# countertype/brotli-lib

Measured on AMD Instinct MI355X. Metric: encode+decode MB/s at q11 lgwin=22, higher is better.
Workload: dtype u8; 1 GPU; C4 per-GPU shard: 1024 x 1048576 B enwik-style text, q11 lgwin22 GENERIC, encode -> decode round trip (statuses and sizes checked); streams_per_gpu=1024, quality=11, lgwin=22, mode=0, parallelism=shard1

## Files before the change

brotli-lib_amd/csrc/enc_common.h:

```cpp
#pragma once
#include <hip/hip_runtime.h>
#include <stdint.h>

#include "common.h"
#include "parts.h"

#ifndef RFC_CONST
#define RFC_CONST static __device__ const
#endif
#include "rfc_tables.h"

namespace mib {
namespace enc {

constexpr uint32_t kSegBits = 16;
constexpr uint32_t kSeg = 1u << kSegBits;
#ifndef MIB_MAX_MATCHES
#define MIB_MAX_MATCHES 4
#endif
constexpr int kMaxMatches = MIB_MAX_MATCHES;
static_assert(kMaxMatches == 4 || kMaxMatches == 6 || kMaxMatches == 8, "records of 4, 6 or 8 entries");
constexpr int kMatchRec = kMaxMatches;
constexpr uint32_t kMatchLenSat = 255;
constexpr int kLongCopy = 200;
// ... 387 lines not shown
                         const uint8_t *dict_data, uint32_t *matches);
void launch_cdict_matches(hipStream_t st, const Job *jobs, const uint32_t *pos_job, uint32_t total, uint32_t *matches);
void launch_find_matches(hipStream_t st, const Job *jobs, const uint32_t *pos_job, const SegRef *seg_ref,
                         const uint32_t *skeys, const uint32_t *svals, uint32_t total, int depth, uint32_t max_dist,
                         bool hist, bool parts, uint32_t *matches);
void launch_near_matches(hipStream_t st, const Job *jobs, const uint32_t *pos_job, const SegRef *seg_ref, uint32_t total,
                         uint32_t max_dist, bool hist, bool parts, uint32_t *matches);
void launch_lit_histo(hipStream_t st, const Job *jobs, const Seg *segs, int nsegs, uint32_t *lit_h);
void launch_hist_update(hipStream_t st, const Job *jobs, const uint32_t *pos_job, const uint32_t *skeys,
                        const uint32_t *svals, uint32_t total);
size_t cost_model_hist_bytes(int njobs);
void launch_cost_model(hipStream_t st, const Job *jobs, int njobs, const Seg *segs, int nsegs, const RawCmd *raw,
                       uint32_t *hist, CostModel *model);
void launch_dp(hipStream_t st, const Job *jobs, const Seg *segs, int nsegs, const uint32_t *lit_h, const CostModel *model,
               const uint32_t *matches, uint64_t *choice, bool cdict, bool font, const uint32_t *words, uint32_t *ring_hist,
               const Mb *mbs);
size_t dp_ring_hist_bytes(int nsegs);
void launch_any_binary(hipStream_t st, const Job *jobs, int njobs, uint32_t *flag);
void launch_words(hipStream_t st, const Job *jobs, const uint32_t *pos_job, const SegRef *seg_ref, uint32_t total, uint32_t *words);
void launch_backtrack(hipStream_t st, const Job *jobs, Seg *segs, int nsegs, const uint64_t *choice, RawCmd *raw);
void launch_carry(hipStream_t st, Job *jobs, int njobs, Seg *segs, const Mb *mbs);
void launch_derive_segs(hipStream_t st, const Seg *segs, int nsegs, uint32_t sample, Seg *d_sample, Seg *pieces);
void launch_merge_pieces(hipStream_t st, const Job *jobs, Seg *segs, int nsegs, const Seg *pieces, RawCmd *raw);
void launch_rep(hipStream_t st, const Job *jobs, Seg *segs, int nsegs, const CostModel *model, RawCmd *raw, uint32_t *cnts);
size_t sort_ws_bytes(uint32_t total);
void launch_sort(hipStream_t st, const Job *jobs, const uint32_t *pos_job, int njobs, uint32_t total, int hb, void *ws,
                 uint32_t *tmp_k, uint32_t *tmp_v, uint32_t *skeys, uint32_t *svals);
void launch_codes(hipStream_t st, const Job *jobs, const Seg *segs, const Mb *mbs, int nsegs, const RawCmd *raw, Cmd *cmds,
                  uint32_t *cmd_pos, Unit *units, uint32_t *unit_h);
void launch_split(hipStream_t st, hipStream_t side, const Job *jobs, Mb *mbs, int nmbs, Unit *units,
                  const uint32_t *unit_h, Codes *codes, int max_units, int max_short_units);
// ... 25 lines not shown
```

brotli-lib_amd/csrc/enc_parse.hip:

```cpp
#include <hipcub/hipcub.hpp>
#include <cstdlib>

#include "enc_common.h"

namespace mib {
namespace enc {

#ifdef MIB_PROF
__device__ unsigned long long g_dp_prof[8];
#define DPMARK(slot)                                  \
  do {                                                \
    const uint64_t t_ = __builtin_amdgcn_s_memtime(); \
    prof[slot] += t_ - pt0;                           \
    pt0 = t_;                                         \
  } while (0)
#define DPCOUNT(slot, v) prof[slot] += (v)
#else
#define DPMARK(slot) do {} while (0)
#define DPCOUNT(slot, v) do {} while (0)
#endif
constexpr int kDpWaves = 4;
constexpr int kLenTab = kLongCopy + 1;
constexpr int kInsTab = 256;
constexpr float kInf = 3.0e38f;
constexpr uint32_t kCostLast = 255;
#ifndef MIB_DP_OCC
#define MIB_DP_OCC 4
#endif
constexpr int kDpWavesPerSimd = MIB_DP_OCC;
#ifndef MIB_DP_OCC_KS4
#define MIB_DP_OCC_KS4 MIB_DP_OCC
#endif
constexpr int kPtabW = 20;
constexpr int kRepLen = 16;
static_assert(kLongCopy <= 325, "copy codes of lengths <= 325 are < 20 (command.ts getCopyLengthCode)");

typedef const __attribute__((address_space(1))) uint8_t GCU8;

__device__ __forceinline__ uint32_t copy_extra(int cc) { return cc < 8 ? 0u : cc < 18 ? (uint32_t)(cc - 6) >> 1 : cc < 23 ? (uint32_t)(cc - 12) : 24u; }
__device__ __forceinline__ uint32_t ins_extra(int ic) {
  return ic < 6 ? 0u : ic < 16 ? (uint32_t)(ic - 4) >> 1 : ic < 21 ? (uint32_t)(ic - 10) : ic == 21 ? 12u : ic == 22 ? 14u : 24u;
}
__device__ __forceinline__ float cmd_cost(int cmd) { return __builtin_amdgcn_logf(11.f + (float)cmd); }
__device__ __forceinline__ float dist_sym_cost(uint32_t code) { return __builtin_amdgcn_logf(20.f + (float)min(code, 127u)); }
__device__ __forceinline__ float cmd_price(int cmd, const CostModel *cm) { return cm ? cm->cmd[cmd] : cmd_cost(cmd); }
__device__ __forceinline__ float dist_price(uint32_t code, const CostModel *cm) {
  return cm ? cm->dist[min(code, 127u)] : dist_sym_cost(code);
// ... 41 lines not shown
__device__ __forceinline__ uint64_t choice_of(uint32_t d, uint32_t m) {
  const uint32_t cl = (m >> 16) ? 0u : m & 0xFFFF;
  return cl ? (((uint64_t)d << 32) | cl) : 0ull;
}
__device__ __forceinline__ uint32_t bperm(uint32_t lane_src, uint32_t v) {
  return (uint32_t)__builtin_amdgcn_ds_bpermute((int)(lane_src << 2), (int)v);
}
__device__ __forceinline__ uint32_t quad_entry0(uint32_t v) { return (uint32_t)__builtin_amdgcn_mov_dpp((int)v, 0x00, 0xF, 0xF, false); }
__device__ __forceinline__ uint32_t quad_entry1(uint32_t v) { return (uint32_t)__builtin_amdgcn_mov_dpp((int)v, 0x55, 0xF, 0xF, false); }
__device__ __forceinline__ uint32_t quad_shift1(uint32_t v) { return (uint32_t)__builtin_amdgcn_mov_dpp((int)v, 0x90, 0xF, 0xF, false); }

constexpr uint32_t kHistPos = 256;
static_assert(kHistPos > (uint32_t)kLongCopy, "a copy's predecessor must still be in the ring history");

template <int KS, bool KM, bool KD, bool KR, bool KC>
__global__ __launch_bounds__(64 * kDpWaves, KS == 4 ? MIB_DP_OCC_KS4 : (KC && KS == 2) ? 3 : kDpWavesPerSimd) void dp_kernel(const Job *jobs, const Seg *segs, int nsegs,
                                                           const uint32_t *lit_histo, const CostModel *model,
                                                           const uint32_t *matches,
                                                           uint64_t *choice , float cmd_pen, int use_rep,
                                                           const uint32_t *pwords, uint32_t *ring_hist, const Mb *mbs,
                                                           int kc_split) {
  constexpr int kS = KS;
  constexpr int kL = 64 / kS;
  constexpr int kC = (kL - 1 + kLongCopy) / kL + 1;
  static_assert(kL - 1 + kLongCopy < kL * kC, "every relaxed length must land in a chunk");
  static_assert(kRepLen <= kL, "a last-distance copy is measured by one lane per byte");
  static_assert(!KC || kL >= 16, "a lane per distance-cache candidate");
  constexpr uint64_t kLaneMask = kL == 64 ? ~0ull : ((1ull << kL) - 1);
  __shared__ uint32_t ptab_all[kDpWaves * kS][24 * kPtabW];
  __shared__ uint8_t cct_all[kL + kLenTab];
  uint8_t *const cctab = cct_all + kL;
  __shared__ uint16_t itab[kInsTab];
  __shared__ uint16_t litc_all[kDpWaves * kS][256];
  constexpr int kPadSh = KS == 4 ? 4 : 5;
  __shared__ StageEnt stg_all[kDpWaves][64 + (64 >> kPadSh)];
  for (int t = (int)threadIdx.x - kL; t < kLenTab; t += 64 * kDpWaves) cctab[t] = (uint8_t)(t >= 2 ? copy_code((uint32_t)t) : 0);
  for (int t = threadIdx.x; t < kInsTab; t += 64 * kDpWaves) {
    const int ic = ins_code((uint32_t)t);
    itab[t] = (uint16_t)(ic | (ins_extra(ic) << 8));
  }
  __syncthreads();
  const uint32_t lane = threadIdx.x & 63, w = (uint32_t)__builtin_amdgcn_readfirstlane((int)(threadIdx.x >> 6));
  const uint32_t h = lane / kL, hl = lane % kL, hbase = h * kL;
  const int sgi = (blockIdx.x * kDpWaves + (int)w) * kS + (int)h;
  StageEnt *stg = stg_all[w];
  uint16_t *litc = litc_all[w * kS + h];
  uint32_t *ptab = ptab_all[w * kS + h];
  uint32_t a = 0, b = 0, gbase = 0, job = 0;
  const uint8_t *data = nullptr;
  int ndirect = 0, npostfix = 0;
  uint32_t parts = 0, abs0 = 0, wabs = 0, pbits = 16, plag = 0, maxback = 0, cdl = 0;
  bool words = false;
  if (sgi < nsegs) {
    const Seg &sg = segs[sgi];
    const Job &jb = jobs[sg.job];
    a = sg.start;
    b = sg.end;
    gbase = jb.pos_base;
    job = sg.job;
    data = jb.data;
    ndirect = (int)jb.ndirect;
    npostfix = (int)jb.npostfix;
    parts = jb.parts;
    abs0 = jb.abs_base;
    wabs = jb.win_abs;
    pbits = jb.part_bits;
    plag = jb.part_lag;
    maxback = (1u << jb.lgwin) - 16;
    words = jb.dict != 0;
    cdl = jb.cdict ? jb.cdict_len : 0u;
  }
  if (kc_split && a < b && (mbs[segs[sgi].mb].ctx_mode == 2u) == KC) a = b;
  if (__ballot(a < b) == 0) return;
  const CostModel *cm = (KM && a < b) ? model + job : nullptr;
  const float dist0 = dist_price(0, cm);
  if (a < b)
    for (uint32_t t = hl; t < 24 * kPtabW; t += kL) {
      const int ic = (int)(t / kPtabW), cc = (int)(t % kPtabW);
      const _Float16 x = (_Float16)(copy_price(ic, cc, false, dist0, cm) + cmd_pen),
                     y = (_Float16)(copy_price(ic, cc, true, dist0, cm) + cmd_pen);
      ptab[t] = (uint32_t)__builtin_bit_cast(uint16_t, x) | ((uint32_t)__builtin_bit_cast(uint16_t, y) << 16);
    }
  if (cm) {
    if (a < b)
      for (uint32_t k = hl; k < 256; k += kL)
        litc[k] = (uint16_t)(uint32_t)(fminf(fmaxf(cm->lit[k], 1.f), 255.f) * 256.f);
  } else {
    uint32_t part = 0;
    if (a < b)
      for (uint32_t k = hl; k < 256; k += kL) part += lit_histo[job * 256 + k];
    for (int o = kL / 2; o; o >>= 1) part += __shfl_xor(part, o);
    const float lt = log2f((float)max(part, 1u));
    if (a < b)
      for (uint32_t k = hl; k < 256; k += kL) {
        const uint32_t c = lit_histo[job * 256 + k];
        const float v = c ? lt - log2f((float)c) : lt + 2.f;
        litc[k] = (uint16_t)(uint32_t)(fminf(fmaxf(v, 1.f), 255.f) * 256.f);
      }
  }
  wave_sync();
  float wc[kC];
  uint32_t wd[kC], wm[kC];
#pragma unroll
  for (int c = 0; c < kC; c++) {
    wc[c] = kInf;
    wd[c] = wm[c] = 0;
  }
  if (hl == 0) wc[0] = 0.f;
  Staged pf;
  uint32_t pf_at = a;
  if (a + hl < b) load_staged<KC>(pf, matches, data, pwords, gbase + a + hl, a + hl);
  uint32_t chd = 0, chm = 0;
  uint32_t rp_d = 0, rp_ic = 0, rp_cb = 0, rp_sb = 1;
  float rp_base = 0.f;
  const uint32_t cj = hl & 15u, rq = hl & 3u;
  const bool clane = KC && hl < 16u && (!KR || cj != 0u);
  const float ccost = KC ? dist_price(cj, cm) : 0.f;
  const uint32_t hoff = (uint32_t)sgi * (kHistPos * 4);
  uint32_t kf = 0;
  uint32_t kp_ld = 0, kp_h = 0;
  float kp_base = 0.f;
  uint32_t rg = 0;
// ... 3 lines not shown
  float cq_base = 0.f;
  auto words_on_ring = [&](uint32_t dd) { return words && is_dict(dd); };
  auto ring_step = [&](uint32_t kind, uint32_t dd, uint32_t h, uint32_t prev) -> uint32_t {
    const uint32_t v = kind == 2u ? h : prev;
    const uint32_t v0 = quad_entry0(v), vm = quad_shift1(v);
    const bool word = words_on_ring(dd);
    const bool push = kind == 2u && dd != v0 && !word;
    return push ? (rq == 0u ? dd : vm) : (kind == 2u && word && rq == 0u) ? dd : v;
  };
  uint32_t i = a, i0 = a;
  bool done = a >= b;
#ifdef MIB_PROF
  uint64_t prof[8] = {0, 0, 0, 0, 0, 0, 0, 0};
  uint64_t pt0 = __builtin_amdgcn_s_memtime();
#endif
  constexpr bool kEarly = KS == 4;
  auto stage = [&]() {
    Staged cur;
#pragma unroll
    for (int q = 0; q < kMaxMatches; q++) cur.m[q] = 0;
    cur.lit = 0;
    cur.w0 = cur.w1 = 0;
    if (pf_at == i0) {
      cur = pf;
    } else if (i0 + hl < b) {
      load_staged<KC>(cur, matches, data, pwords, gbase + i0 + hl, i0 + hl);
    }
    const uint32_t nx = i0 + kL;
    if constexpr (!kEarly) {
      if (nx + hl < b) load_staged<KC>(pf, matches, data, pwords, gbase + nx + hl, nx + hl);
    }
// ... 49 lines not shown
#pragma unroll
    for (int q = 0; kEarly && q < kMaxMatches; q++)
      if ((uint32_t)q < nm) {
        const float dc = (float)(dpq[q] >> 10) + dsc[q];
        e.mc[q] |= min((uint32_t)(dc * 4.f + 0.5f), kCostLast - 1) << 24;
      }
    e.info = (maxlen ? nm : 0u) | (maxlen << 8) | ((word ? maxlen : 2u) << 16);
    e.w[0] = KC ? cur.w0 : 0u;
    e.w[1] = KC ? cur.w1 : 0u;
    stg[lane + (lane >> kPadSh)] = e;
    if constexpr (kEarly) {
      if (nx + hl < b) load_staged<KC>(pf, matches, data, pwords, gbase + nx + hl, nx + hl);
    }
    pf_at = nx;
  };
  constexpr int kPre = kEarly ? 3 : 0;
  struct StepIn {
    uint32_t info;
    float lc;
    uint32_t m[kMaxMatches], mc[kMaxMatches];
    uint32_t cc[kPre ? kPre : 1];
  };
  auto read_step = [&](uint32_t o) {
    const uint32_t s = hbase + (o & (kL - 1));
    const StageEnt &e = stg[s + (s >> kPadSh)];
    StepIn r;
    r.info = e.info;
    r.lc = e.lc;
    if constexpr (kMaxMatches == 4) {
      const uint4 em = *reinterpret_cast<const uint4 *>(e.m), emc = *reinterpret_cast<const uint4 *>(e.mc);
      r.m[0] = em.x; r.m[1] = em.y; r.m[2] = em.z; r.m[3] = em.w;
// ... 93 lines not shown
          const uint32_t p = i0 + hl;
          if (p <= i && p != a) choice[gbase + p] = choice_of(chd, chm);
        }
        if (KC) {
          const uint32_t r1 = (kf & 3u) ? ring_step(kf & 3u, kp_ld, kp_h, rg) : rg;
          const bool ccopy = !(kf & 4u) && mm >= 2u && (mm >> 16) == 0u;
          const uint32_t hv = ccopy ? ring_hist[hoff + ((i - mm) & (kHistPos - 1)) * 4 + rq] : 0u;
          const uint32_t ri = ring_step(ccopy ? 2u : 1u, ld, hv, r1);
          rg = ring_step(2u, fd, ri, ri);
          kf = 4u;
        }
        i += fl;
        i0 = i;
        rp_d = 0;
#pragma unroll
        for (int c = 0; c < kC; c++) wc[c] = kInf;
        if (hl == 0) {
          wc[0] = fc;
          wd[0] = fd;
          wm[0] = fl;
        }
        stage();
      }
      wave_sync();
      DPMARK(2);
      continue;
    }
    const uint32_t actm = 0u - (uint32_t)act;
    uint32_t mL[kMaxMatches], vpk[kMaxMatches];
#pragma unroll
    for (int q = 0; q < kMaxMatches; q++) {
      mL[q] = match_length(e.m[q]) & actm;
      vpk[q] = e.mc[q];
    }
    uint32_t R = 0;
    if (KR) {
      const uint64_t eqm = (__ballot(rp_cb == rp_sb) >> hbase) & ((1ull << kRepLen) - 1);
      R = (act && rp_d) ? (eqm == (1ull << kRepLen) - 1 ? (uint32_t)kRepLen : (uint32_t)__ffsll((unsigned long long)~eqm) - 1u) : 0u;
      if (parts && R) R = min(R, part_cap(abs0 + i - 1, rp_d, pbits, plag));
      R = R >= 2 ? R : 0u;
    }
    const uint32_t maxrel = max(max(1u, maxlen), R ? R - 1 : 0u);

#pragma unroll
    for (int c = 0; c < kC; c++) {
      if (c > 0 && __ballot(act && (uint32_t)(kL * c) <= off + maxrel) == 0) break;
      const uint32_t l = (uint32_t)(kL * c) + hl - off;
      float cand = kInf;
      uint32_t nd = ld, nmeta = (ins1 << 16) | nx;
      if (l == 1 && act) cand = ci + litcost;
      if (l >= minlen && l <= maxlen) {
        uint32_t x = 0;
#pragma unroll
        for (int q = kMaxMatches - 1; q >= 0; q--)
          x = l <= mL[q] ? vpk[q] : x;
        const uint32_t tv = c < kPre ? tvp[c] : trow[cctab[l]];
        const float pn = (float)__builtin_bit_cast(_Float16, (uint16_t)(tv & 0xFFFF));
        const float pl = (float)__builtin_bit_cast(_Float16, (uint16_t)(tv >> 16));
        nd = match_dist(x);
        if (KD && nd == kCDictMark) nd = min(wabs + i, maxback) + l;
        const float alt = __builtin_fmaf((float)(x >> 24), 0.25f, pn);
        const uint32_t use_last = 0u - (uint32_t)(nd == ld);
        cand = base + __uint_as_float((__float_as_uint(pl) & use_last) | (__float_as_uint(alt) & ~use_last));
        nmeta = l;
      }
      if (cand < wc[c]) {
        wc[c] = cand;
        wd[c] = nd;
        wm[c] = nmeta;
      }
    }
    if (KR && __ballot(R != 0)) {
      const uint32_t *rrow = ptab + rp_ic * kPtabW;
#pragma unroll
      for (int c = 0; c < 2 && c < kC; c++) {
        const uint32_t lr = (uint32_t)(kL * c) + hl - off + 1u;
        if (lr >= 2u && lr <= R) {
          const uint32_t tv = rrow[cctab[lr]];
          const float cr = rp_base + (float)__builtin_bit_cast(_Float16, (uint16_t)(tv >> 16));
          if (cr < wc[c]) {
            wc[c] = cr;
            wd[c] = rp_d;
            wm[c] = lr;
          }
        }
      }
    }
    if (KR) {
      const bool rv = act && use_rep && ins > 0 && ld != 0u && !(words && is_dict(ld)) && ld <= min(wabs + i, maxback);
      rp_d = rv ? ld : 0u;
// ... 10 lines not shown
    if (KC) {
      const uint32_t x0 = cq_w0 ^ cq_c0, x1 = cq_w1 ^ cq_c1;
      uint32_t R = x0 ? 0u : x1 ? 4u + ((uint32_t)__builtin_ctz(x1) >> 3) : 8u;
      if (__ballot(R == 8u && cq_d != 0u)) {
        uint32_t full = 0;
#pragma unroll
        for (int q = 0; q < kMaxMatches; q++) full = match_dist(cq_m[q]) == cq_d ? max(full, match_length(cq_m[q])) : full;
        R = R == 8u ? max(R, full) : R;
      }
      R = min(R, cq_lim);
      const bool pass = act && (kf & 8u) && cq_d != 0u && R >= 4u;
      uint64_t pm = __ballot(pass);
      DPCOUNT(2, pm ? 1 : 0);
      if (pm) {
        const uint32_t *crow = ptab + ((kf >> 16) & 0xFFu) * kPtabW;
        uint32_t ctv[kC];
#pragma unroll
        for (int c = 0; c < kC; c++) {
          ctv[c] = 0u;
          if (c > 1 && __ballot(pass && (uint32_t)(kL * c) + 2u <= off + R) == 0) break;
          const uint32_t lr = (uint32_t)(kL * c) + hl + 2u - off;
          if (lr >= 4u && lr <= (uint32_t)kLongCopy) ctv[c] = crow[cctab[lr]];
        }
        do {
          const uint32_t mine = (uint32_t)((pm >> hbase) & 0xFFFFull);
          const uint32_t k = mine ? (uint32_t)__builtin_ctz(mine) : 0u;
          const uint32_t src = hbase + k;
          const uint32_t Rk = mine ? bperm(src, R) : 0u, dk = bperm(src, cq_d);
          const float ck = __uint_as_float(bperm(src, __float_as_uint(ccost)));
#pragma unroll
          for (int c = 0; c < kC; c++) {
            if (c > 1 && __ballot((uint32_t)(kL * c) + 2u <= off + Rk) == 0) break;
            const uint32_t lr = (uint32_t)(kL * c) + hl + 2u - off;
            if (lr >= 4u && lr <= Rk) {
              const float cr = cq_base + (k ? (float)__builtin_bit_cast(_Float16, (uint16_t)(ctv[c] & 0xFFFF)) + ck
                                            : (float)__builtin_bit_cast(_Float16, (uint16_t)(ctv[c] >> 16)));
              if (cr < wc[c]) {
                wc[c] = cr;
                wd[c] = dk;
                wm[c] = lr;
              }
            }
          }
          pm &= ~__ballot(mine != 0u && hl == k);
          DPCOUNT(7, 1);
        } while (pm);
// ... 24 lines not shown
      kf = (act ? (ccopy ? 2u : 1u) : 0u) | (pk ? 8u : 0u) | ((uint32_t)ic << 8) | (((kf >> 8) & 0xFFu) << 16);
      kp_ld = ld;
      kp_base = base;
      if (cv) {
        cq_w0 = pwords[cx - cq_d];
        cq_w1 = pwords[cx - cq_d + 4u];
        cq_c0 = pwords[cx];
        cq_c1 = pwords[cx + 4u];
        rec_load(matches + (uint64_t)cx * kMatchRec, cq_m);
      }
    }
    DPMARK(5);
    if (act) i++;
    const bool bend = act && i - i0 == (uint32_t)kL;
    if (__ballot(bend)) {
#pragma unroll
      for (int c = 0; c + 1 < kC; c++) {
        wc[c] = bend ? wc[c + 1] : wc[c];
        wd[c] = bend ? wd[c + 1] : wd[c];
        wm[c] = bend ? wm[c + 1] : wm[c];
      }
      wc[kC - 1] = bend ? kInf : wc[kC - 1];
      wd[kC - 1] = bend ? 0u : wd[kC - 1];
      wm[kC - 1] = bend ? 0u : wm[kC - 1];
      if (bend) {
        if (i0 + hl != a) choice[gbase + i0 + hl] = choice_of(chd, chm);
        i0 = i;
        stage();
      }
      wave_sync();
    }
    DPMARK(3);
  }
#ifdef MIB_PROF
  if (lane == 0)
    for (int q = 0; q < 8; q++) atomicAdd(&g_dp_prof[q], (unsigned long long)prof[q]);
#endif
}

// ... 447 lines not shown
  if (t == 0) sg.ncmd = n + chunk_split[nch];
}
void launch_rep(hipStream_t st, const Job *jobs, Seg *segs, int nsegs, const CostModel *model, RawCmd *raw, uint32_t *cnts) {
  if (nsegs) hipLaunchKernelGGL(rep_kernel, dim3(nsegs), dim3(kRepT), 0, st, jobs, segs, model, raw, cnts);
}

#ifdef MIB_PROF
extern "C" int mib_debug_read_dp_prof(unsigned long long *out) {
  hipMemcpyFromSymbol(out, HIP_SYMBOL(g_dp_prof), sizeof(unsigned long long) * 8);
  unsigned long long z[8] = {0, 0, 0, 0, 0, 0, 0, 0};
  hipMemcpyToSymbol(HIP_SYMBOL(g_dp_prof), z, sizeof(z));
  return 0;
}
#endif
constexpr int kKs4Segs = 3 * 4 * 1024;
static int dp_ks(int nsegs, bool font) {
  static const int v = knob("MIB_DP_KS") ? atoi(knob("MIB_DP_KS")) : 0;
  if (v == 1 || v == 2 || v == 4) return v;
  return !font && nsegs >= kKs4Segs ? 4 : nsegs <= 2048 ? 1 : 2;
}
template <bool KD, bool KC>
static void launch_dp_t(hipStream_t st, const Job *jobs, const Seg *segs, int nsegs, const uint32_t *lit_h,
                        const CostModel *model, const uint32_t *matches, uint64_t *choice, bool font,
                        const uint32_t *words, uint32_t *ring_hist, const Mb *mbs, int kc_split) {
  const int ks = dp_ks(nsegs, font), spw = kDpWaves * ks;
  const dim3 g((nsegs + spw - 1) / spw), b(64 * kDpWaves);
  static const float cmd_pen = knob("MIB_CMD_PENALTY") ? (float)atof(knob("MIB_CMD_PENALTY")) : 0.f;
  static const int rep_knob = knob("MIB_DP_REP") ? atoi(knob("MIB_DP_REP")) : 1;
  const bool rep = rep_knob == 2 || (rep_knob == 1 && font);
#define MIB_DP(K, M, R) \
  hipLaunchKernelGGL((dp_kernel<K, M, KD, R, KC>), g, b, 0, st, jobs, segs, nsegs, lit_h, model, matches, choice, cmd_pen, 1, words, ring_hist, mbs, kc_split)
#define MIB_DP_KS(K)                \
  do {                              \
    if (model && rep) MIB_DP(K, true, true);   \
    else if (model) MIB_DP(K, true, false);    \
    else if (rep) MIB_DP(K, false, true);      \
    else MIB_DP(K, false, false);              \
  } while (0)
  if (ks == 1) MIB_DP_KS(1);
  else if (ks == 4) MIB_DP_KS(4);
  else MIB_DP_KS(2);
#undef MIB_DP_KS
#undef MIB_DP
}
void launch_dp(hipStream_t st, const Job *jobs, const Seg *segs, int nsegs, const uint32_t *lit_h, const CostModel *model,
               const uint32_t *matches, uint64_t *choice, bool cdict, bool font, const uint32_t *words, uint32_t *ring_hist,
               const Mb *mbs) {
  const bool kc = words && ring_hist && mbs;
  if (cdict) {
    if (kc) launch_dp_t<true, true>(st, jobs, segs, nsegs, lit_h, model, matches, choice, font, words, ring_hist, mbs, 1);
    launch_dp_t<true, false>(st, jobs, segs, nsegs, lit_h, model, matches, choice, font, words, ring_hist, mbs, kc ? 1 : 0);
  } else {
    if (kc) launch_dp_t<false, true>(st, jobs, segs, nsegs, lit_h, model, matches, choice, font, words, ring_hist, mbs, 1);
    launch_dp_t<false, false>(st, jobs, segs, nsegs, lit_h, model, matches, choice, font, words, ring_hist, mbs, kc ? 1 : 0);
  }
}
size_t dp_ring_hist_bytes(int nsegs) { return (size_t)std::max(nsegs, 1) * kHistPos * 16; }
__global__ void words_kernel(const Job *jobs, const uint32_t *pos_job, const SegRef *seg_ref, uint32_t total, uint32_t *words) {
  const uint32_t g = blockIdx.x * blockDim.x + threadIdx.x;
  if (g >= total || !jobs[pos_job[g >> kSegBits]].binary) return;
  const SegRef r = seg_ref[g >> kSegBits];
  uint32_t v = 0;
#pragma unroll
  for (uint32_t k = 0; k < 4; k++)
    if (g + k < r.end) v |= (uint32_t)r.base[g + k] << (8 * k);
  words[g] = v;
}
__global__ void any_binary_kernel(const Job *jobs, int njobs, uint32_t *flag) {
  uint32_t v = 0;
  for (int j = threadIdx.x; j < njobs; j += blockDim.x) v |= jobs[j].binary;
// ... 23 lines not shown
```

brotli-lib_amd/csrc/encode.hip:

```cpp
#include <hip/hip_runtime.h>
#include <stdio.h>
#include <stdlib.h>
#include <string.h>

#include <algorithm>
#include <atomic>
#include <memory>
#include <mutex>
#include <thread>
#include <vector>

#include "enc_common.h"

extern "C" void mib_ctx_add_time(mib_ctx *c, const char *name, double ms);
extern "C" int mib_ctx_profiling(mib_ctx *c);
extern "C" void **mib_ctx_enc_ws(mib_ctx *c);
extern "C" void **mib_ctx_lane_ws(mib_ctx *c, int l);
extern "C" void *mib_ctx_lane_stream(mib_ctx *c, int l);
extern "C" uint8_t *mib_ctx_stage(mib_ctx *c, int slot, uint64_t need);

using namespace mib;
using namespace mib::enc;

extern "C" mib_ctx *mib_default_ctx(void);
// ... 256 lines not shown
    return nullptr;
  }
  d.data = dd;
  d.tab = dt;
  return &d;
}

int encode_group(mib_ctx *ctx, const Params &prm, const StreamDesc *sd, size_t k, uint8_t *d_out, uint64_t out_cap,
                 uint64_t out_pos, uint64_t *sizes, int32_t (*dc_out)[4], hipStream_t st, void **ws_slot) {
  std::vector<Job> jobs(k);
  std::vector<Seg> segs;
  std::vector<Mb> mbs;
  std::vector<uint32_t> seg_job;
  std::vector<SegRef> seg_ref;
  uint64_t pos_total = 0, out_scratch = 0, cmd_total = 0, npieces = 0;
  bool any_hist = false, any_parts = false, any_dict = false, any_cdict = false;
  for (size_t j = 0; j < k; j++) {
    Job &jb = jobs[j];
    memset(&jb, 0, sizeof(jb));
    const uint64_t n = sd[j].n;
    jb.data = sd[j].d_data;
    jb.n = (uint32_t)n;
    jb.lgwin = (uint32_t)prm.lgwin;
    jb.npostfix = (uint32_t)prm.npostfix;
    jb.ndirect = (uint32_t)prm.ndirect;
    jb.uncompressed = (prm.quality == 0 || n < 64) ? 1 : 0;
    jb.font = prm.font ? 1 : 0;
    jb.hq = prm.quality >= 10 ? 1 : 0;
    jb.hdr_lgwin = sd[j].hdr_lgwin;
    jb.final_ = sd[j].final_;
// ... 39 lines not shown
        mb.end = (uint32_t)std::min<uint64_t>(n, m0 + mb_max);
        mb.first_seg = (uint32_t)segs.size();
        mb.is_last = (mb.end == n && jb.final_) ? 1 : 0;
        for (uint64_t s0 = m0; s0 < mb.end; s0 += kSeg) {
          Seg sg;
          memset(&sg, 0, sizeof(sg));
          sg.job = (uint32_t)j;
          sg.start = (uint32_t)s0;
          sg.end = (uint32_t)std::min<uint64_t>(mb.end, s0 + kSeg);
          sg.mb = (uint32_t)mbs.size();
          sg.cmd_off = (uint32_t)cmd_total;
          cmd_total += (sg.end - sg.start) / 2 + 4 + (2 << kMaxPieceShift);
          const int pshift = dp_piece_shift(n, sd[j].streaming);
          sg.pieces = (uint32_t)(npieces << 3) | (uint32_t)pshift;
          npieces += 1ull << pshift;
          segs.push_back(sg);
        }
        mb.nseg = (uint32_t)segs.size() - mb.first_seg;
        mbs.push_back(mb);
      }
    }
    jb.nseg = (uint32_t)segs.size() - jb.seg_base;
    jb.nmb = (uint32_t)mbs.size() - jb.mb_base;
    const uint64_t span = ((n + kSeg - 1) / kSeg) * kSeg + kSeg;
    for (uint64_t q = 0; q < span / kSeg; q++) {
      seg_job.push_back((uint32_t)j);
      seg_ref.push_back(SegRef{jb.data - (uintptr_t)pos_total, (uint32_t)pos_total, (uint32_t)(pos_total + (jb.uncompressed ? 0 : n))});
    }
    pos_total += span;
    jb.out_off = out_scratch;
// ... 139 lines not shown
      uint32_t any = 0;
      CK(hipMemcpyAsync(&any, d_any_binary, 4, hipMemcpyDeviceToHost, st));
      CK(hipStreamSynchronize(st));
      if (any) {
        launch_words(st, d_jobs, d_seg_job, d_seg_ref, total, pos_words);
      } else {
        pos_words = nullptr;
        ring_hist = nullptr;
      }
    }
    fk.fork();
    if (forked && any_hist) launch_hist_update(fk.side, d_jobs, d_seg_job, skeys, svals, total);
    tm.start(two_pass ? "dp_sample" : "dp_parse");
    Seg *s1 = sampled ? d_sample : two_pass ? d_segs : d_fin;
    const int n1 = s1 == d_fin ? nfin : nsegs;
    launch_dp(st, d_jobs, s1, n1, lit_h, nullptr, matches, choice, any_cdict, prm.font, pos_words, ring_hist, d_mbs);
    tm.stop();
    tm.start("backtrack");
    launch_backtrack(st, d_jobs, s1, n1, choice, raw);
    tm.stop();
    if (two_pass) {
      tm.start("cost_model");
      launch_cost_model(st, d_jobs, (int)k, s1, nsegs, raw, model_h, model);
      tm.stop();
      tm.start("dp_parse");
      launch_dp(st, d_jobs, d_fin, nfin, lit_h, model, matches, choice, any_cdict, prm.font, pos_words, ring_hist, d_mbs);
      tm.stop();
      tm.start("backtrack");
      launch_backtrack(st, d_jobs, d_fin, nfin, choice, raw);
      tm.stop();
    }
    if (ps) launch_merge_pieces(st, d_jobs, d_segs, nsegs, d_pieces, raw);
    tm.start("codes");
    launch_carry(st, d_jobs, (int)k, d_segs, d_mbs);
    if (two_pass && rep_pass(prm)) launch_rep(st, d_jobs, d_segs, nsegs, model, raw, cmd_pos);
    launch_ring_scan(st, d_jobs, (int)k, d_segs, nsegs, raw, push);
    launch_codes(st, d_jobs, d_segs, d_mbs, nsegs, raw, cmds, cmd_pos, units, unit_h);
    launch_dist_ring(st, d_jobs, (int)k, d_segs, cmds);
    tm.stop();
    tm.start("block_split");
    fk.fork();
// ... 238 lines not shown
  uint8_t *buf[2] = {nullptr, nullptr};
  uint64_t buf_cap = 0;
  int cur = 0;
  uint64_t hist = 0;
  uint64_t abs = 0;
  uint64_t obytes = 0;
  uint32_t *tab = nullptr;
  std::vector<uint8_t> dict;
  DevDict ddict;
  uint8_t *stage = nullptr;
  uint64_t staged = 0;
};
extern "C" {

void mib_force_no_dp_cache(int off) { __atomic_store_n(&g_no_dp_cache, off ? 1 : 0, __ATOMIC_RELAXED); }

void mib_encode_ws_free(void *p) {
  Workspace *ws = reinterpret_cast<Workspace *>(p);
  if (!ws) return;
  if (ws->buf) hipFree(ws->buf);
  if (ws->side) hipStreamDestroy(ws->side);
  if (ws->fork_ev) hipEventDestroy(ws->fork_ev);
  if (ws->join_ev) hipEventDestroy(ws->join_ev);
  delete ws;
}
int mib_live_encoders(void) { return g_live_encoders.load(); }
void mib_encode_ws_trim(void **p, uint64_t keep) {
  Workspace *ws = reinterpret_cast<Workspace *>(*p);
  if (!ws) return;
  ws->quiet = ws->need > keep ? 0 : ws->quiet + 1;
// ... 449 lines not shown
```

brotli-lib_amd/python/brotli_amd/__init__.py:

```python
import ctypes
import os

__all__ = ['brotliEncode', 'BrotliEncoder', 'brotliDecode', 'BrotliDecoder', 'brotliDecodedSize', 'EncoderMode', 'BrotliError',
           'encode_batch', 'decode_batch', 'encoder_update_batch', 'decoder_update_batch', 'decoder_finish_batch',
           'decoder_update_batch_device', 'decoder_finish_batch_device', 'MORE_OUTPUT', 'DeviceContext', 'library_path']

_PKG = os.path.dirname(os.path.dirname(os.path.dirname(os.path.abspath(__file__))))
_LIB_PATH = os.environ.get('BROTLI_AMD_LIB') or os.path.join(_PKG, 'libbrotli_amd.so')


def library_path():
    return _LIB_PATH


class EncoderMode:
    GENERIC = 0
    TEXT = 1
    FONT = 2


class BrotliError(Exception):
    def __init__(self, message, code=None):
        super().__init__(message)
        self.code = code
# ... 433 lines not shown
    outs = (_Buf * k)()
    st = (ctypes.c_int * k)()
    if gpus is None:
        rc = _L().mib_encode_batch(spans, k, ctypes.byref(_opts(options)), outs, st)
    else:
        rc = _L().mib_encode_batch_n(spans, k, ctypes.byref(_opts(options)), int(gpus), outs, st)
    if rc:
        raise _err(rc)
    res = [_take(outs[i]) for i in range(k)]
    for i in range(k):
        if st[i]:
            raise _err(st[i])
    return res


def debug_match_records(buffers, options=None):
    import numpy as np
    k = len(buffers)
    keep = [_in(b) for b in buffers]
    spans = (_Span * k)(*[_Span(_addr(a), n) for a, n, _ in keep])
    outs = (_Buf * k)()
    rc = _L().mib_debug_match_records(spans, k, ctypes.byref(_opts(options)), outs)
    if rc:
        raise _err(rc)
    res = []
    for i in range(k):
        n = keep[i][1]
        a = np.frombuffer(_take(outs[i]), dtype='<u4')
        res.append(a.reshape(n, -1) if n else a.reshape(0, 4))
    return res
# ... 129 lines not shown
```

include/brotli_amd.h:

```cpp
#ifndef BROTLI_AMD_H_
#define BROTLI_AMD_H_
#include <stddef.h>
#include <stdint.h>
#ifdef __cplusplus
extern "C" {
#endif

#define MIB_MODE_GENERIC 0
#define MIB_MODE_TEXT 1
#define MIB_MODE_FONT 2

#define MIB_E_NO_DEVICE (-100)
#define MIB_E_INVALID_ARG (-101)
#define MIB_E_OUT_OF_MEMORY (-102)
#define MIB_E_OUTPUT_LIMIT (-103)
#define MIB_E_NEED_SPACE (-104)
#define MIB_E_JS_RANGE_ERROR (-105)
#define MIB_E_JS_TYPE_ERROR (-106)
#define MIB_E_NO_PROGRESS (-107)

typedef struct {
  int quality;
  int lgwin;
  int mode;
// ... 50 lines not shown
uint64_t mib_decoder_held_output(const mib_decoder *d);
int mib_debug_copy_batch(const uint8_t *const *d_src, uint8_t *const *d_dst, const uint64_t *n, size_t k);
void mib_decoder_batch_stats(uint64_t *launches);
void mib_decoder_batch_times(double *ms, int n);
void mib_force_decoder_grid(int max_blocks);

int mib_encode_batch(const mib_span *in, size_t k, const mib_enc_opts *o, mib_buf *out, int *status);
int mib_decode_batch(const mib_span *in, size_t k, mib_buf *out, int *status);
int mib_encode_batch_n(const mib_span *in, size_t k, const mib_enc_opts *o, int n_gpus, mib_buf *out, int *status);
int mib_decode_batch_n(const mib_span *in, size_t k, int n_gpus, mib_buf *out, int *status);
int mib_device_count(void);
int64_t mib_selftest_lds_atomic_order(int trials);
void mib_force_ballot_rank(int force);
void mib_force_shards(int force);
void mib_force_no_dp_cache(int off);
int mib_debug_match_records(const mib_span *in, size_t k, const mib_enc_opts *o, mib_buf *out);

void mib_buf_free(mib_buf *b);
typedef void *(*mib_alloc_func)(void *opaque, size_t size);
typedef void (*mib_free_func)(void *opaque, void *address);
void mib_set_allocator(mib_alloc_func alloc_func, mib_free_func free_func, void *opaque);

typedef struct mib_ctx mib_ctx;
mib_ctx *mib_ctx_new(int device);
void mib_ctx_free(mib_ctx *c);
int mib_ctx_encode(mib_ctx *c, const mib_enc_opts *o, const uint8_t *d_in, const uint64_t *in_offsets,
                   size_t k, uint8_t *d_out, uint64_t out_cap, uint64_t *out_offsets, void *stream);
int mib_ctx_decode(mib_ctx *c, const uint8_t *d_in, const uint64_t *in_offsets, size_t k, uint8_t *d_out,
                   const uint64_t *out_offsets, int64_t *out_sizes, int *status, void *stream);
typedef struct { char name[32]; double ms; uint32_t launches; } mib_kernel_time;
// ... 18 lines not shown
```

Measured before the change: 3369 MB/s.

## Add eight-pieces-per-wave DP variant with LDS-spilled far window ring

```diff
diff --git a/brotli-lib_amd/csrc/enc_common.h b/brotli-lib_amd/csrc/enc_common.h
--- a/brotli-lib_amd/csrc/enc_common.h
+++ b/brotli-lib_amd/csrc/enc_common.h
@@ -425,7 +425,8 @@
                        uint32_t *hist, CostModel *model);
 void launch_dp(hipStream_t st, const Job *jobs, const Seg *segs, int nsegs, const uint32_t *lit_h, const CostModel *model,
                const uint32_t *matches, uint64_t *choice, bool cdict, bool font, const uint32_t *words, uint32_t *ring_hist,
-               const Mb *mbs);
+               const Mb *mbs, int piece_shift);
+void dp_launch_counts(unsigned long long out[4]);
 size_t dp_ring_hist_bytes(int nsegs);
 void launch_any_binary(hipStream_t st, const Job *jobs, int njobs, uint32_t *flag);
 void launch_words(hipStream_t st, const Job *jobs, const uint32_t *pos_job, const SegRef *seg_ref, uint32_t total, uint32_t *words);
diff --git a/brotli-lib_amd/csrc/enc_parse.hip b/brotli-lib_amd/csrc/enc_parse.hip
--- a/brotli-lib_amd/csrc/enc_parse.hip
+++ b/brotli-lib_amd/csrc/enc_parse.hip
@@ -31,6 +31,8 @@
 #ifndef MIB_DP_OCC_KS4
 #define MIB_DP_OCC_KS4 MIB_DP_OCC
 #endif
+constexpr int kNear8 = 12;
+constexpr int kPre8 = 4;
 constexpr int kPtabW = 20;
 constexpr int kRepLen = 16;
 static_assert(kLongCopy <= 325, "copy codes of lengths <= 325 are < 20 (command.ts getCopyLengthCode)");
@@ -102,26 +104,33 @@
 static_assert(kHistPos > (uint32_t)kLongCopy, "a copy's predecessor must still be in the ring history");
 
 template <int KS, bool KM, bool KD, bool KR, bool KC>
-__global__ __launch_bounds__(64 * kDpWaves, KS == 4 ? MIB_DP_OCC_KS4 : (KC && KS == 2) ? 3 : kDpWavesPerSimd) void dp_kernel(const Job *jobs, const Seg *segs, int nsegs,
+__global__ __launch_bounds__(64 * kDpWaves, KS == 8 ? 3 : KS == 4 ? MIB_DP_OCC_KS4 : (KC && KS == 2) ? 3 : kDpWavesPerSimd) void dp_kernel(const Job *jobs, const Seg *segs, int nsegs,
                                                            const uint32_t *lit_histo, const CostModel *model,
                                                            const uint32_t *matches,
                                                            uint64_t *choice , float cmd_pen, int use_rep,
                                                            const uint32_t *pwords, uint32_t *ring_hist, const Mb *mbs,
                                                            int kc_split) {
   constexpr int kS = KS;
+  constexpr bool KW = KS == 8;
   constexpr int kL = 64 / kS;
   constexpr int kC = (kL - 1 + kLongCopy) / kL + 1;
   static_assert(kL - 1 + kLongCopy < kL * kC, "every relaxed length must land in a chunk");
-  static_assert(kRepLen <= kL, "a last-distance copy is measured by one lane per byte");
+  constexpr int kW = KS == 8 ? kNear8 : kC;
+  constexpr int kFar = kC - kW;
+  static_assert(KS == 8 || kFar == 0, "the other builds keep the whole window in registers");
+  static_assert(!KR || kRepLen <= kL, "a last-distance copy is measured by one lane per byte");
+  static_assert(KS < 8 || (!KD && !KR && !KC), "eight pieces a wave: the plain build only");
+  constexpr int kT = KW ? 1 : kS;
   static_assert(!KC || kL >= 16, "a lane per distance-cache candidate");
   constexpr uint64_t kLaneMask = kL == 64 ? ~0ull : ((1ull << kL) - 1);
-  __shared__ uint32_t ptab_all[kDpWaves * kS][24 * kPtabW];
+  __shared__ uint32_t ptab_all[kDpWaves * kT][24 * kPtabW];
   __shared__ uint8_t cct_all[kL + kLenTab];
   uint8_t *const cctab = cct_all + kL;
   __shared__ uint16_t itab[kInsTab];
-  __shared__ uint16_t litc_all[kDpWaves * kS][256];
-  constexpr int kPadSh = KS == 4 ? 4 : 5;
+  __shared__ uint16_t litc_all[kDpWaves * kT][256];
+  constexpr int kPadSh = KS == 8 ? 3 : KS == 4 ? 4 : 5;
   __shared__ StageEnt stg_all[kDpWaves][64 + (64 >> kPadSh)];
+  __shared__ uint2 far_all[kDpWaves][kFar ? kFar * 64 : 1];
   for (int t = (int)threadIdx.x - kL; t < kLenTab; t += 64 * kDpWaves) cctab[t] = (uint8_t)(t >= 2 ? copy_code((uint32_t)t) : 0);
   for (int t = threadIdx.x; t < kInsTab; t += 64 * kDpWaves) {
     const int ic = ins_code((uint32_t)t);
@@ -132,8 +141,8 @@
   const uint32_t h = lane / kL, hl = lane % kL, hbase = h * kL;
   const int sgi = (blockIdx.x * kDpWaves + (int)w) * kS + (int)h;
   StageEnt *stg = stg_all[w];
-  uint16_t *litc = litc_all[w * kS + h];
-  uint32_t *ptab = ptab_all[w * kS + h];
+  uint16_t *litc = litc_all[KW ? w : w * kS + h];
+  uint32_t *ptab = ptab_all[KW ? w : w * kS + h];
   uint32_t a = 0, b = 0, gbase = 0, job = 0;
   const uint8_t *data = nullptr;
   int ndirect = 0, npostfix = 0;
@@ -162,38 +171,54 @@
   if (__ballot(a < b) == 0) return;
   const CostModel *cm = (KM && a < b) ? model + job : nullptr;
   const float dist0 = dist_price(0, cm);
-  if (a < b)
-    for (uint32_t t = hl; t < 24 * kPtabW; t += kL) {
+  constexpr uint32_t kF = KW ? 64u : (uint32_t)kL;
+  const uint32_t tl = KW ? lane : hl;
+  uint32_t fjob = job;
+  bool fill = a < b;
+  if constexpr (KW) {
+    fjob = (uint32_t)__builtin_amdgcn_readlane((int)job, (int)__ffsll((unsigned long long)__ballot(a < b)) - 1);
+    fill = true;
+  }
+  const CostModel *cmf = KW ? (KM ? model + fjob : nullptr) : cm;
+  const float dist0f = KW ? dist_price(0, cmf) : dist0;
+  if (fill)
+    for (uint32_t t = tl; t < 24 * kPtabW; t += kF) {
       const int ic = (int)(t / kPtabW), cc = (int)(t % kPtabW);
-      const _Float16 x = (_Float16)(copy_price(ic, cc, false, dist0, cm) + cmd_pen),
-                     y = (_Float16)(copy_price(ic, cc, true, dist0, cm) + cmd_pen);
+      const _Float16 x = (_Float16)(copy_price(ic, cc, false, dist0f, cmf) + cmd_pen),
+                     y = (_Float16)(copy_price(ic, cc, true, dist0f, cmf) + cmd_pen);
       ptab[t] = (uint32_t)__builtin_bit_cast(uint16_t, x) | ((uint32_t)__builtin_bit_cast(uint16_t, y) << 16);
     }
-  if (cm) {
-    if (a < b)
-      for (uint32_t k = hl; k < 256; k += kL)
-        litc[k] = (uint16_t)(uint32_t)(fminf(fmaxf(cm->lit[k], 1.f), 255.f) * 256.f);
+  if (cmf) {
+    if (fill)
+      for (uint32_t k = tl; k < 256; k += kF)
+        litc[k] = (uint16_t)(uint32_t)(fminf(fmaxf(cmf->lit[k], 1.f), 255.f) * 256.f);
   } else {
     uint32_t part = 0;
-    if (a < b)
-      for (uint32_t k = hl; k < 256; k += kL) part += lit_histo[job * 256 + k];
-    for (int o = kL / 2; o; o >>= 1) part += __shfl_xor(part, o);
+    if (fill)
+      for (uint32_t k = tl; k < 256; k += kF) part += lit_histo[fjob * 256 + k];
+    for (int o = (int)kF / 2; o; o >>= 1) part += __shfl_xor(part, o);
     const float lt = log2f((float)max(part, 1u));
-    if (a < b)
-      for (uint32_t k = hl; k < 256; k += kL) {
-        const uint32_t c = lit_histo[job * 256 + k];
+    if (fill)
+      for (uint32_t k = tl; k < 256; k += kF) {
+        const uint32_t c = lit_histo[fjob * 256 + k];
         const float v = c ? lt - log2f((float)c) : lt + 2.f;
         litc[k] = (uint16_t)(uint32_t)(fminf(fmaxf(v, 1.f), 255.f) * 256.f);
       }
   }
   wave_sync();
-  float wc[kC];
-  uint32_t wd[kC], wm[kC];
-#pragma unroll
-  for (int c = 0; c < kC; c++) {
+  float wc[kW];
+  uint32_t wd[kW], wm[kW];
+#pragma unroll
+  for (int c = 0; c < kW; c++) {
     wc[c] = kInf;
     wd[c] = wm[c] = 0;
   }
+  uint2 *const far = far_all[w] + lane;
+  uint32_t fbase = 0;
+  auto far_clear = [&]() {
+    for (int s2 = 0; s2 < kFar; s2++) far[64 * s2] = make_uint2(__float_as_uint(kInf), 0u);
+  };
+  if constexpr (kFar > 0) far_clear();
   if (hl == 0) wc[0] = 0.f;
   Staged pf;
   uint32_t pf_at = a;
@@ -227,7 +252,7 @@
   uint64_t prof[8] = {0, 0, 0, 0, 0, 0, 0, 0};
   uint64_t pt0 = __builtin_amdgcn_s_memtime();
 #endif
-  constexpr bool kEarly = KS == 4;
+  constexpr bool kEarly = KS >= 4;
   auto stage = [&]() {
     Staged cur;
 #pragma unroll
@@ -307,7 +332,7 @@
     }
     pf_at = nx;
   };
-  constexpr int kPre = kEarly ? 3 : 0;
+  constexpr int kPre = KS == 8 ? kPre8 : kEarly ? 3 : 0;
   struct StepIn {
     uint32_t info;
     float lc;
@@ -431,7 +456,8 @@
         i0 = i;
         rp_d = 0;
 #pragma unroll
-        for (int c = 0; c < kC; c++) wc[c] = kInf;
+        for (int c = 0; c < kW; c++) wc[c] = kInf;
+        if constexpr (kFar > 0) far_clear();
         if (hl == 0) {
           wc[0] = fc;
           wd[0] = fd;
@@ -460,7 +486,7 @@
     const uint32_t maxrel = max(max(1u, maxlen), R ? R - 1 : 0u);
 
 #pragma unroll
-    for (int c = 0; c < kC; c++) {
+    for (int c = 0; c < kW; c++) {
       if (c > 0 && __ballot(act && (uint32_t)(kL * c) <= off + maxrel) == 0) break;
       const uint32_t l = (uint32_t)(kL * c) + hl - off;
       float cand = kInf;
@@ -487,10 +513,34 @@
         wm[c] = nmeta;
       }
     }
+    if constexpr (kFar > 0) {
+      if (__ballot(act && (uint32_t)(kL * kW) <= off + maxrel)) {
+        for (int c = kW; c < kC; c++) {
+          if (__ballot(act && (uint32_t)(kL * c) <= off + maxrel) == 0) break;
+          const uint32_t l = (uint32_t)(kL * c) + hl - off;
+          if (l >= minlen && l <= maxlen) {
+            uint32_t x = 0;
+#pragma unroll
+            for (int q = kMaxMatches - 1; q >= 0; q--)
+              x = l <= mL[q] ? vpk[q] : x;
+            const uint32_t tv = trow[cctab[l]];
+            const float pn = (float)__builtin_bit_cast(_Float16, (uint16_t)(tv & 0xFFFF));
+            const float pl = (float)__builtin_bit_cast(_Float16, (uint16_t)(tv >> 16));
+            const uint32_t nd = match_dist(x);
+            const float alt = __builtin_fmaf((float)(x >> 24), 0.25f, pn);
+            const float cand = base + (nd == ld ? pl : alt);
+            uint32_t s2 = fbase + (uint32_t)(c - kW);
+            s2 = s2 >= (uint32_t)kFar ? s2 - (uint32_t)kFar : s2;
+            const uint2 cur = far[64 * s2];
+            if (cand < __uint_as_float(cur.x)) far[64 * s2] = make_uint2(__float_as_uint(cand), nd | (l << 24));
+          }
+        }
+      }
+    }
     if (KR && __ballot(R != 0)) {
       const uint32_t *rrow = ptab + rp_ic * kPtabW;
 #pragma unroll
-      for (int c = 0; c < 2 && c < kC; c++) {
+      for (int c = 0; c < 2 && c < kW; c++) {
         const uint32_t lr = (uint32_t)(kL * c) + hl - off + 1u;
         if (lr >= 2u && lr <= R) {
           const uint32_t tv = rrow[cctab[lr]];
@@ -531,9 +581,9 @@
       DPCOUNT(2, pm ? 1 : 0);
       if (pm) {
         const uint32_t *crow = ptab + ((kf >> 16) & 0xFFu) * kPtabW;
-        uint32_t ctv[kC];
-#pragma unroll
-        for (int c = 0; c < kC; c++) {
+        uint32_t ctv[kW];
+#pragma unroll
+        for (int c = 0; c < kW; c++) {
           ctv[c] = 0u;
           if (c > 1 && __ballot(pass && (uint32_t)(kL * c) + 2u <= off + R) == 0) break;
           const uint32_t lr = (uint32_t)(kL * c) + hl + 2u - off;
@@ -546,7 +596,7 @@
           const uint32_t Rk = mine ? bperm(src, R) : 0u, dk = bperm(src, cq_d);
           const float ck = __uint_as_float(bperm(src, __float_as_uint(ccost)));
 #pragma unroll
-          for (int c = 0; c < kC; c++) {
+          for (int c = 0; c < kW; c++) {
             if (c > 1 && __ballot((uint32_t)(kL * c) + 2u <= off + Rk) == 0) break;
             const uint32_t lr = (uint32_t)(kL * c) + hl + 2u - off;
             if (lr >= 4u && lr <= Rk) {
@@ -601,15 +651,34 @@
     if (act) i++;
     const bool bend = act && i - i0 == (uint32_t)kL;
     if (__ballot(bend)) {
-#pragma unroll
-      for (int c = 0; c + 1 < kC; c++) {
-        wc[c] = bend ? wc[c + 1] : wc[c];
-        wd[c] = bend ? wd[c + 1] : wd[c];
-        wm[c] = bend ? wm[c + 1] : wm[c];
-      }
-      wc[kC - 1] = bend ? kInf : wc[kC - 1];
-      wd[kC - 1] = bend ? 0u : wd[kC - 1];
-      wm[kC - 1] = bend ? 0u : wm[kC - 1];
+      uint32_t bmask = bend ? ~0u : 0u;
+      if constexpr (KW) asm("" : "+v"(bmask));
+#pragma unroll
+      for (int c = 0; c + 1 < kW; c++) {
+        if constexpr (KW) {
+          wc[c] = __uint_as_float((__float_as_uint(wc[c + 1]) & bmask) | (__float_as_uint(wc[c]) & ~bmask));
+          wd[c] = (wd[c + 1] & bmask) | (wd[c] & ~bmask);
+          wm[c] = (wm[c + 1] & bmask) | (wm[c] & ~bmask);
+        } else {
+          wc[c] = bend ? wc[c + 1] : wc[c];
+          wd[c] = bend ? wd[c + 1] : wd[c];
+          wm[c] = bend ? wm[c + 1] : wm[c];
+        }
+      }
+      if constexpr (kFar > 0) {
+        const uint2 nxt = far[64 * fbase];
+        wc[kW - 1] = bend ? __uint_as_float(nxt.x) : wc[kW - 1];
+        wd[kW - 1] = bend ? (nxt.y & 0xFFFFFFu) : wd[kW - 1];
+        wm[kW - 1] = bend ? (nxt.y >> 24) : wm[kW - 1];
+        if (bend) {
+          far[64 * fbase] = make_uint2(__float_as_uint(kInf), 0u);
+          fbase = fbase + 1u == (uint32_t)kFar ? 0u : fbase + 1u;
+        }
+      } else {
+        wc[kC - 1] = bend ? kInf : wc[kC - 1];
+        wd[kC - 1] = bend ? 0u : wd[kC - 1];
+        wm[kC - 1] = bend ? 0u : wm[kC - 1];
+      }
       if (bend) {
         if (i0 + hl != a) choice[gbase + i0 + hl] = choice_of(chd, chm);
         i0 = i;
@@ -1087,22 +1156,31 @@
 }
 #endif
 constexpr int kKs4Segs = 3 * 4 * 1024;
-static int dp_ks(int nsegs, bool font) {
+constexpr int kKs8Segs = 8704;
+static int dp_ks(int nsegs, bool font, bool plain, int piece_shift) {
   static const int v = knob("MIB_DP_KS") ? atoi(knob("MIB_DP_KS")) : 0;
+  const bool can8 = !font && plain && piece_shift >= 3;
+  if (v == 8 && can8) return 8;
   if (v == 1 || v == 2 || v == 4) return v;
+  if (can8 && nsegs >= kKs8Segs) return 8;
   return !font && nsegs >= kKs4Segs ? 4 : nsegs <= 2048 ? 1 : 2;
 }
+static unsigned long long g_dp_launches[4];
 template <bool KD, bool KC>
 static void launch_dp_t(hipStream_t st, const Job *jobs, const Seg *segs, int nsegs, const uint32_t *lit_h,
                         const CostModel *model, const uint32_t *matches, uint64_t *choice, bool font,
-                        const uint32_t *words, uint32_t *ring_hist, const Mb *mbs, int kc_split) {
-  const int ks = dp_ks(nsegs, font), spw = kDpWaves * ks;
-  const dim3 g((nsegs + spw - 1) / spw), b(64 * kDpWaves);
-  static const float cmd_pen = knob("MIB_CMD_PENALTY") ? (float)atof(knob("MIB_CMD_PENALTY")) : 0.f;
+                        const uint32_t *words, uint32_t *ring_hist, const Mb *mbs, int kc_split, int piece_shift) {
   static const int rep_knob = knob("MIB_DP_REP") ? atoi(knob("MIB_DP_REP")) : 1;
   const bool rep = rep_knob == 2 || (rep_knob == 1 && font);
+  const bool plain = !KD && !KC && !rep;
+  const int ks = dp_ks(nsegs, font, plain, piece_shift), spw = kDpWaves * ks;
+  const dim3 g((nsegs + spw - 1) / spw), b(64 * kDpWaves);
+  __atomic_fetch_add(&g_dp_launches[ks == 8 ? 3 : ks == 4 ? 2 : ks == 2 ? 1 : 0], 1ull, __ATOMIC_RELAXED);
+  static const float cmd_pen = knob("MIB_CMD_PENALTY") ? (float)atof(knob("MIB_CMD_PENALTY")) : 0.f;
 #define MIB_DP(K, M, R) \
   hipLaunchKernelGGL((dp_kernel<K, M, KD, R, KC>), g, b, 0, st, jobs, segs, nsegs, lit_h, model, matches, choice, cmd_pen, 1, words, ring_hist, mbs, kc_split)
+#define MIB_DP_8(M) \
+  hipLaunchKernelGGL((dp_kernel<8, M, false, false, false>), g, b, 0, st, jobs, segs, nsegs, lit_h, model, matches, choice, cmd_pen, 1, words, ring_hist, mbs, kc_split)
 #define MIB_DP_KS(K)                \
   do {                              \
     if (model && rep) MIB_DP(K, true, true);   \
@@ -1110,23 +1188,30 @@
     else if (rep) MIB_DP(K, false, true);      \
     else MIB_DP(K, false, false);              \
   } while (0)
-  if (ks == 1) MIB_DP_KS(1);
+  if (ks == 8) {
+    if (model) MIB_DP_8(true);
+    else MIB_DP_8(false);
+  } else if (ks == 1) MIB_DP_KS(1);
   else if (ks == 4) MIB_DP_KS(4);
   else MIB_DP_KS(2);
 #undef MIB_DP_KS
+#undef MIB_DP_8
 #undef MIB_DP
 }
 void launch_dp(hipStream_t st, const Job *jobs, const Seg *segs, int nsegs, const uint32_t *lit_h, const CostModel *model,
                const uint32_t *matches, uint64_t *choice, bool cdict, bool font, const uint32_t *words, uint32_t *ring_hist,
-               const Mb *mbs) {
+               const Mb *mbs, int piece_shift) {
   const bool kc = words && ring_hist && mbs;
   if (cdict) {
-    if (kc) launch_dp_t<true, true>(st, jobs, segs, nsegs, lit_h, model, matches, choice, font, words, ring_hist, mbs, 1);
-    launch_dp_t<true, false>(st, jobs, segs, nsegs, lit_h, model, matches, choice, font, words, ring_hist, mbs, kc ? 1 : 0);
+    if (kc) launch_dp_t<true, true>(st, jobs, segs, nsegs, lit_h, model, matches, choice, font, words, ring_hist, mbs, 1, piece_shift);
+    launch_dp_t<true, false>(st, jobs, segs, nsegs, lit_h, model, matches, choice, font, words, ring_hist, mbs, kc ? 1 : 0, piece_shift);
   } else {
-    if (kc) launch_dp_t<false, true>(st, jobs, segs, nsegs, lit_h, model, matches, choice, font, words, ring_hist, mbs, 1);
-    launch_dp_t<false, false>(st, jobs, segs, nsegs, lit_h, model, matches, choice, font, words, ring_hist, mbs, kc ? 1 : 0);
-  }
+    if (kc) launch_dp_t<false, true>(st, jobs, segs, nsegs, lit_h, model, matches, choice, font, words, ring_hist, mbs, 1, piece_shift);
+    launch_dp_t<false, false>(st, jobs, segs, nsegs, lit_h, model, matches, choice, font, words, ring_hist, mbs, kc ? 1 : 0, piece_shift);
+  }
+}
+void dp_launch_counts(unsigned long long out[4]) {
+  for (int q = 0; q < 4; q++) out[q] = __atomic_load_n(&g_dp_launches[q], __ATOMIC_RELAXED);
 }
 size_t dp_ring_hist_bytes(int nsegs) { return (size_t)std::max(nsegs, 1) * kHistPos * 16; }
 __global__ void words_kernel(const Job *jobs, const uint32_t *pos_job, const SegRef *seg_ref, uint32_t total, uint32_t *words) {
diff --git a/brotli-lib_amd/csrc/encode.hip b/brotli-lib_amd/csrc/encode.hip
--- a/brotli-lib_amd/csrc/encode.hip
+++ b/brotli-lib_amd/csrc/encode.hip
@@ -294,6 +294,7 @@
   std::vector<uint32_t> seg_job;
   std::vector<SegRef> seg_ref;
   uint64_t pos_total = 0, out_scratch = 0, cmd_total = 0, npieces = 0;
+  int min_pshift = kMaxPieceShift;
   bool any_hist = false, any_parts = false, any_dict = false, any_cdict = false;
   for (size_t j = 0; j < k; j++) {
     Job &jb = jobs[j];
@@ -363,6 +364,7 @@
           const int pshift = dp_piece_shift(n, sd[j].streaming);
           sg.pieces = (uint32_t)(npieces << 3) | (uint32_t)pshift;
           npieces += 1ull << pshift;
+          min_pshift = std::min(min_pshift, pshift);
           segs.push_back(sg);
         }
         mb.nseg = (uint32_t)segs.size() - mb.first_seg;
@@ -532,7 +534,8 @@
     tm.start(two_pass ? "dp_sample" : "dp_parse");
     Seg *s1 = sampled ? d_sample : two_pass ? d_segs : d_fin;
     const int n1 = s1 == d_fin ? nfin : nsegs;
-    launch_dp(st, d_jobs, s1, n1, lit_h, nullptr, matches, choice, any_cdict, prm.font, pos_words, ring_hist, d_mbs);
+    launch_dp(st, d_jobs, s1, n1, lit_h, nullptr, matches, choice, any_cdict, prm.font, pos_words, ring_hist, d_mbs,
+              s1 == d_fin && ps ? min_pshift : 0);
     tm.stop();
     tm.start("backtrack");
     launch_backtrack(st, d_jobs, s1, n1, choice, raw);
@@ -542,7 +545,8 @@
       launch_cost_model(st, d_jobs, (int)k, s1, nsegs, raw, model_h, model);
       tm.stop();
       tm.start("dp_parse");
-      launch_dp(st, d_jobs, d_fin, nfin, lit_h, model, matches, choice, any_cdict, prm.font, pos_words, ring_hist, d_mbs);
+      launch_dp(st, d_jobs, d_fin, nfin, lit_h, model, matches, choice, any_cdict, prm.font, pos_words, ring_hist, d_mbs,
+                ps ? min_pshift : 0);
       tm.stop();
       tm.start("backtrack");
       launch_backtrack(st, d_jobs, d_fin, nfin, choice, raw);
@@ -811,6 +815,11 @@
 extern "C" {
 
 void mib_force_no_dp_cache(int off) { __atomic_store_n(&g_no_dp_cache, off ? 1 : 0, __ATOMIC_RELAXED); }
+void mib_debug_dp_launches(uint64_t out[4]) {
+  unsigned long long v[4];
+  enc::dp_launch_counts(v);
+  for (int q = 0; q < 4; q++) out[q] = v[q];
+}
 
 void mib_encode_ws_free(void *p) {
   Workspace *ws = reinterpret_cast<Workspace *>(p);
diff --git a/brotli-lib_amd/python/brotli_amd/__init__.py b/brotli-lib_amd/python/brotli_amd/__init__.py
--- a/brotli-lib_amd/python/brotli_amd/__init__.py
+++ b/brotli-lib_amd/python/brotli_amd/__init__.py
@@ -471,6 +471,12 @@
     return res
 
 
+def debug_dp_launches():
+    out = (ctypes.c_uint64 * 4)()
+    _L().mib_debug_dp_launches(out)
+    return {1: out[0], 2: out[1], 4: out[2], 8: out[3]}
+
+
 def debug_match_records(buffers, options=None):
     import numpy as np
     k = len(buffers)
diff --git a/include/brotli_amd.h b/include/brotli_amd.h
--- a/include/brotli_amd.h
+++ b/include/brotli_amd.h
@@ -88,6 +88,7 @@
 void mib_force_ballot_rank(int force);
 void mib_force_shards(int force);
 void mib_force_no_dp_cache(int off);
+void mib_debug_dp_launches(uint64_t out[4]);
 int mib_debug_match_records(const mib_span *in, size_t k, const mib_enc_opts *o, mib_buf *out);
 
 void mib_buf_free(mib_buf *b);
```

Result: faster. 3529 MB/s (median of 6 runs) (+4.7%).
